# mpieva/mapping-iterative-assembler

Measured on AMD Instinct MI355X. Metric: reads aligned/sec per iteration (16.5kb mito ref, 100bp reads), higher is better.
Workload: dtype int32; 1 GPU; configs[1]: 1000000 synthetic 100 bp reads per GPU vs mt311 (16619 bp, circular), matrix flat; step = reiterate_assembly + pop_smp + cull + consensus; pass-1 coordinates = true positions; reads_per_gpu=1000000, total_reads=1000000, consensus_len=16619, bytes_per_read=182

## Files before the change

mapping-iterative-assembler_amd/csrc/mia_consensus_kernels.h:

```cpp
#pragma once
#include <hip/hip_runtime.h>
#include <stdint.h>

#include "ma_records.h"
#include "mia_kernels.h"
#include "mia_layout.h"

namespace mia {

struct TallyBuf {
  int32_t* tally;
  int32_t Lp;
  int32_t* gaps;
  uint64_t* events;
  int32_t* n_events;
  int32_t cap_events;
  uint32_t* flags;
};

struct RecGeom {
  int start_w, end, split, ncols_f, ncols_b;
};
MIA_HD inline RecGeom rec_geom(int as, int ae, int L) {
  RecGeom g;
// ... 684 lines not shown
        for (int m = 0; m < mult; m++) {
          int slot = BINNED ? atomicAdd(ev_cnt, 1) : TALLY_EV_CAP;
          if (slot < TALLY_EV_CAP) ev_buf[slot] = ev;
          else {
            const int e = atomicAdd(tb.n_events, 1);
            if (e < tb.cap_events) tb.events[e] = ev; else atomicOr(tb.flags, 1u);
          }
        }
      }
    }
  }
}

__global__ __launch_bounds__(256) void k_tally(ReadSet rs, RefInfo ref, const int32_t* pssm2, const uint8_t* drop_front,
                                                const uint8_t* drop_back, TallyBuf tb, const int32_t* rec_params, const int32_t* rec_actf) {
  const int lane = threadIdx.x & 63;
  const int64_t i = (int64_t)blockIdx.x * 4 + (threadIdx.x >> 6);
  if (i >= rs.n) return;
  tally_one_read<false>(__builtin_amdgcn_readfirstlane((int)i), lane, rs, ref, pssm2, drop_front, drop_back, tb, nullptr, 0, rec_params, rec_actf, nullptr, nullptr, nullptr);
}

constexpr int BUCKET_PER = 8;
__device__ __forceinline__ int bucket_of(const ReadSet& rs, int64_t i, int nb, int split) {
  return (min(rs.as[i] / TALLY_BUCKET, (nb >> split) - 1) << split) | (split ? (rs.rc[i] ? 1 : 0) : 0);
}
__device__ __forceinline__ bool bucket_takes(const ReadSet& rs, int64_t i) { return i < rs.n && rs.sk[i]; }
constexpr int SORT2_KEYS = 256;
__device__ __forceinline__ int sort2_key(const ReadSet& rs, int64_t i, int b, int split) {
  if (!(rs.status[i] & ST_DIAG) || rs.abr[i] != 0) return SORT2_KEYS - 1;
  const int k = rs.as[i] - (b >> split) * TALLY_BUCKET;
  return k < 0 ? 0 : (k >= SORT2_KEYS - 1 ? SORT2_KEYS - 2 : k);
}
__global__ __launch_bounds__(256) void k_bucket_count(ReadSet rs, int32_t nb, int32_t* count, int32_t* zero, int64_t zero_words, const int32_t* abort_if = nullptr,
                                                       int32_t split = 0) {
  if (abort_if && *abort_if != 0) return;
  extern __shared__ int32_t hist[];
  for (int b = threadIdx.x; b < nb; b += blockDim.x) hist[b] = 0;
  if (zero) for (int64_t k = (int64_t)blockIdx.x * 256 + threadIdx.x; k < zero_words; k += (int64_t)gridDim.x * 256) zero[k] = 0;
  __syncthreads();
  for (int k = 0; k < BUCKET_PER; k++) {
    const int64_t i = ((int64_t)blockIdx.x * BUCKET_PER + k) * 256 + threadIdx.x;
    if (bucket_takes(rs, i)) atomicAdd(&hist[bucket_of(rs, i, nb, split)], 1);
  }
  __syncthreads();
  for (int b = threadIdx.x; b < nb; b += blockDim.x) if (hist[b]) atomicAdd(&count[b], hist[b]);
}
__global__ __launch_bounds__(256) void k_bucket_scan(int32_t* count, int32_t nb, int32_t* off, int32_t* wgoff, int32_t* cursor, int32_t* wg_bucket, const int32_t* abort_if = nullptr,
                                                      int32_t chunk = TALLY_CHUNK) {
  if (abort_if && *abort_if != 0) return;
  __shared__ int32_t s_run[256], s_wg[256];
  const int t = threadIdx.x, per = (nb + 255) / 256, b0 = t * per, b1 = b0 + per < nb ? b0 + per : nb;
  int run = 0, wg = 0;
  for (int b = b0; b < b1; b++) { run += count[b]; wg += (count[b] + chunk - 1) / chunk; }
  s_run[t] = run; s_wg[t] = wg;
  __syncthreads();
  for (int o = 1; o < 256; o <<= 1) {
    const int a = t >= o ? s_run[t - o] : 0, c = t >= o ? s_wg[t - o] : 0;
    __syncthreads();
    s_run[t] += a; s_wg[t] += c;
    __syncthreads();
  }
  int r = s_run[t] - run, w = s_wg[t] - wg;
  for (int b = b0; b < b1; b++) {
    off[b] = r; wgoff[b] = w; cursor[b] = 0;
    const int cb = count[b];
    const int nw = (cb + chunk - 1) / chunk;
    for (int q = 0; q < nw; q++) reinterpret_cast<int4*>(wg_bucket)[w + q] = make_int4(b, r + q * chunk, min(r + (q + 1) * chunk, r + cb), 0);
    r += cb; w += nw;
    count[b] = 0;
  }
  if (t == 255) { off[nb] = s_run[255]; wgoff[nb] = s_wg[255]; }
// ... 936 lines not shown
      if (code < 4) atomicAdd(&t[(T_A + code) * Lp], 1);
      const int32_t* row = pm + d * 25 + code;
      atomicAdd(&t[T_SA * Lp], row[0]);
      atomicAdd(&t[T_SC * Lp], row[5]);
      atomicAdd(&t[T_SG * Lp], row[10]);
      atomicAdd(&t[T_ST * Lp], row[15]);
    }
    if (p > 0) atomicAdd(&t[T_SPAN * Lp], 1);
  }
}
__global__ void k_ma_ins_events(MaRecords mr, int64_t n_ins, const int32_t* ins_record, const int32_t* ins_pos, const int64_t* ins_off,
                                const char* ins_bases, TallyBuf tb) {
  const int64_t e = (int64_t)blockIdx.x * blockDim.x + threadIdx.x;
  if (e >= n_ins) return;
  const int r = ins_record[e], p = ins_pos[e];
  const int64_t o0 = mr.col_off[r];
  const int ncols = (int)(mr.col_off[r + 1] - o0);
  if (p <= 0 || p >= ncols) return;
  const int gc = mr.start[r] + p, d = (int)mr.smp[o0 + p] - 'A';
  if (gc >= tb.Lp || d < 0 || d > 2 * PSSM_DEPTH) { atomicOr(tb.flags, 2u); return; }
  const int len = (int)(ins_off[e + 1] - ins_off[e]);
  for (int j = 0; j < len && j < 1024; j++) {
    const int code = ma_code(ins_bases[ins_off[e] + j]);
    const int slot = atomicAdd(tb.n_events, 1);
    if (slot < tb.cap_events)
      tb.events[slot] = (uint64_t)(uint32_t)gc | ((uint64_t)j << 32) | ((uint64_t)(code == 5 ? 4 : code) << 42) | ((uint64_t)(d & 31) << 45) |
                        ((uint64_t)(mr.revcom[r] ? 1 : 0) << 50);
    else atomicOr(tb.flags, 1u);
  }
}

MIA_HD inline int64_t ins_words(int64_t cap) { return ((cap * 9 + 1) & ~(int64_t)1) + cap * 6; }
MIA_HD inline unsigned long long* ins_sc_of(int32_t* ins_tally, int64_t cap) { return reinterpret_cast<unsigned long long*>(ins_tally + ((cap * 9 + 1) & ~(int64_t)1)); }
__global__ void k_ins_tally(const uint64_t* events, int32_t n_events, const int32_t* pssm2, const int32_t* ins_off,
                            const int32_t* gaps, int32_t L, int32_t* ins_tally, int32_t cap, const int32_t* n_events_dev, int32_t cap_events, const int32_t* abort_if = nullptr) {
  if (abort_if && *abort_if != 0) return;
  if (n_events_dev) n_events = min(*n_events_dev, cap_events);
  for (int e = blockIdx.x * blockDim.x + threadIdx.x; e < n_events; e += gridDim.x * blockDim.x) {
  const uint64_t ev = events[e];
  const int gc = (int)(uint32_t)ev, j = (int)((ev >> 32) & 1023), code = (int)((ev >> 42) & 7), d = (int)((ev >> 45) & 31);
  const int rc = (int)((ev >> 50) & 1);
  if (gc <= 0 || gc >= L || j >= gaps[gc] || ins_off[gc] + j >= cap) continue;
  const int64_t sl = (int64_t)(ins_off[gc] + j);
  int32_t* t = ins_tally + sl * 9;
  unsigned long long* sc = ins_sc_of(ins_tally, cap) + sl * 3;
  const int32_t* row = pssm2 + (rc ? PSSM_WORDS : 0) + d * 25 + code;
  if (code < 4) atomicAdd(&t[code], 1);
  else atomicAdd(&sc[2], 1ull);
  atomicAdd(&sc[0], (unsigned long long)(((long long)row[5] << 32) + (long long)row[0]));
  atomicAdd(&sc[1], (unsigned long long)(((long long)row[15] << 32) + (long long)row[10]));
  }
}

__device__ __forceinline__ char call_base(int As, int Cs, int Gs, int Ts, int gapsn, int cov, int sA, int sC, int sG, int sT,
                                          int cons_code) {
  (void)As; (void)Cs; (void)Gs; (void)Ts;
  if (cov == 0) return 'N';
  if (((double)gapsn / (double)cov) >= (double)(50 / 100.0)) return '-';
  int top = sA, second = INT32_MIN;
  char base = 'A';
  if (sC >= top) { second = top; top = sC; base = 'C'; } else second = sC;
  if (sG >= top) { second = top; top = sG; base = 'G'; } else if (sG >= second) second = sG;
  if (sT >= top) { second = top; top = sT; base = 'T'; } else if (sT >= second) second = sT;
  if (cons_code == 2) return (top >= 0 || (top - 2400) > second) ? base : 'N';
  return (top >= -399) ? base : 'N';
}

__global__ void k_call_columns(const int32_t* tally, int32_t Lp, int32_t L, int cons_code, char* calls) {
  int p = blockIdx.x * blockDim.x + threadIdx.x;
  if (p >= L) return;
  calls[p] = call_base(tally[T_A * Lp + p], tally[T_C * Lp + p], tally[T_G * Lp + p], tally[T_T * Lp + p],
                       tally[T_GAP * Lp + p], tally[T_COV * Lp + p], tally[T_SA * Lp + p], tally[T_SC * Lp + p],
                       tally[T_SG * Lp + p], tally[T_ST * Lp + p], cons_code);
}
__device__ __forceinline__ void call_inserts_at(int p, const int32_t* tally, int32_t Lp, const int32_t* gaps, const int32_t* ins_off,
                                                int32_t* ins_tally, int cons_code, char* ins_calls, int32_t cap) {
  const int span = tally[T_SPAN * Lp + p];
  for (int j = 0; j < gaps[p] && ins_off[p] + j < cap; j++) {
    const int64_t sl = (int64_t)(ins_off[p] + j);
    int32_t* t = ins_tally + sl * 9;
    const unsigned long long* sc = ins_sc_of(ins_tally, cap) + sl * 3;
    const long long x0 = (long long)sc[0], x1 = (long long)sc[1];
    const int32_t sA = (int32_t)(uint32_t)x0, sC = (int32_t)((x0 - (long long)sA) >> 32), sG = (int32_t)(uint32_t)x1, sT = (int32_t)((x1 - (long long)sG) >> 32);
// ... 14 lines not shown
```

mapping-iterative-assembler_amd/csrc/mia_hip.hip:

```cpp
#include <hip/hip_runtime.h>
#include <atomic>
#include <hip/hip_ext.h>
#include <stdio.h>
#include <stdlib.h>
#include <string.h>

#include <algorithm>
#include <cmath>
#include <chrono>
#include <optional>
#include <string>
#include <thread>
#include <tuple>
#include <vector>

#include "../../include/mia_hip.h"
#include "dev_buf.h"
#include "dev_pool.h"
#include "mia_comm.h"
#include "mia_consensus_kernels.h"
#include "mia_kernels.h"
#include "bandx_kernels.h"
#include "align_route.h"
#include "pass1_route.h"
// ... 15 lines not shown
enum Stage { STG_TRACE = 0, STG_PLAIN, STG_FILTER, STG_BAND, STG_BX_PLAN, STG_BX_VALUES, STG_BX_TRACE, STG_TALLY, STG_PASS1, STG_MA_SELECT, STG_MA_RENDER, STG_MA_ACE_LAYOUT, STG_MA_ACE_RENDER, STG_MA_SAM_LAYOUT, STG_MA_SAM_RENDER, STG_MA_PROFILE, STG_MA_DEDUP_KEYS, STG_MA_DEDUP_SORT, STG_MA_DEDUP_RUNS, STG_MA_DEDUP_NEXT, STG_MA_DEDUP_ANCHORS, STG_MA_DEDUP_CLUSTERS, STG_MA_TALLY, STG_MA_COLS, STG_MA_ENDS, STG_COUNT };
static const char* const STAGE_NAMES[STG_COUNT] = {"k_align_quad", "k_align_quad_plain", "k_diag_filter", "k_band_align", "k_bx_plan",
                                                   "k_bx_values", "k_bx_trace", "k_tally_binned", "k_pass1", "k_ma_region_select",
                                                   "k_ma_region_render", "k_ma_ace_layout", "k_ma_ace_render", "k_ma_sam_layout",
                                                   "k_ma_sam_render", "k_ma_profile", "k_ma_dedup_keys", "k_ma_dedup_sort", "k_ma_dedup_runs",
                                                   "k_ma_dedup_next", "k_ma_dedup_anchors", "k_ma_dedup_clusters", "k_ma_tally", "k_ma_cols", "k_ma_ends"};

constexpr int OPEN_WGS = 1024;
constexpr int64_t OPEN_SLAB_BYTES = (int64_t)MAX_READ * 64 * 12;
constexpr int CTRL_BINS = 0;
constexpr int CTRL_HDR = (3 * N_BINS + 2 + 1) & ~1;
constexpr int CTRL_FILTER = CTRL_HDR + PH_WORDS;
constexpr int CTRL_LKN = CTRL_FILTER + 4, CTRL_CULLF = CTRL_LKN + 1, CTRL_NEV = CTRL_CULLF + 1, CTRL_TFLAGS = CTRL_NEV + 1;
constexpr int CTRL_GENN = CTRL_TFLAGS + 2;
constexpr int CTRL_BXC = (CTRL_GENN + 1 + 63) & ~63;
constexpr int CTRL_WORDS = CTRL_BXC + BXC_WORDS;
constexpr int CTRL_C0 = CTRL_BINS + 3 * N_BINS, CTRL_CN = CTRL_WORDS - CTRL_C0;

#ifdef MIA_HIP_ALT_PATHS
static inline const char* alt_env(const char* name) { return getenv(name); }
#define ALT_KERNEL(k) ((const void*)(k))
#else
static inline const char* alt_env(const char*) { return nullptr; }
#define ALT_KERNEL(k) ((const void*)nullptr)
#endif
static inline std::optional<int> alt_int(const char* name) {
  const char* v = alt_env(name);
  return v ? std::optional<int>(atoi(v)) : std::nullopt;
}

struct mia_hip_ctx {
  int device = 0;
  int cus = 1;
  std::string err;
  DevPool pool;
  unsigned char* h_pin = nullptr; static constexpr size_t PIN_BYTES = 1 << 20, PIN_MISC = 64 << 10;
  DevBuf<int32_t> d_ctrl;
  uint32_t dbg = 0;

  hipStream_t stream = nullptr;
  hipStream_t stream2 = nullptr; hipEvent_t ev_fork = nullptr, ev_join = nullptr;
  hipStream_t stream3 = nullptr; hipEvent_t ev_join3 = nullptr;
  uint32_t ext_events = 31u; bool align_end_signalled = false;
  bool spin_wait = true;
  uint32_t stage_mask = ~0u;
  struct StageTimer { std::vector<std::pair<hipEvent_t, hipEvent_t>> pending; double ms = 0; int64_t launches = 0; };
  StageTimer stg[STG_COUNT];
  std::vector<std::pair<hipEvent_t, hipEvent_t>> ev_free;

  DevBuf<int32_t> d_pssm;
  int max_abs = 0;
  int max_pos = 0;
  bool have_pssm = false;
  bool flat = false;
  PackSet packs;
  ReadSet rs{};
  DevBuf<uint8_t> d_packed; DevBuf<uint32_t> d_roff; DevBuf<uint16_t> d_len;
  DevBuf<uint8_t> d_rc, d_sk;
  DevBuf<int32_t> d_as, d_ae, d_score, d_refstart;
  DevBuf<int16_t> d_abr; DevBuf<uint32_t> d_status; DevBuf<int16_t> d_cols;
  int max_len = 0;
  int min_len = 0;
  std::vector<int32_t> h_len;
  DevBuf<uint64_t> d_rplanes; int rplane_words = 0;
  DevBuf<int32_t> d_umax; bool umax_valid = false;
  DevBuf<uint8_t> d_ref; int L = 0, wrap = 0; int explicit_win = 0; bool have_ref = false; bool aligned = false;
// ... 45 lines not shown
  DevBuf<int32_t> d_retry2;
  bool diag_scripts_missing = false;
  int64_t bx_seen = 0, bx_done[3] = {0, 0, 0};
  int64_t bx_launches = 0;
  uint32_t bx_last[BXC_COUNTERS] = {0};

  DevBuf<int64_t> d_slot, d_partial, d_total;
  DevBuf<uint8_t> d_slot_dropped, d_drop_f, d_drop_b; int64_t n_slots = 0;
  DevBuf<int64_t> d_back_slot;
  DevBuf<int64_t> d_front_slot0;
  DevBuf<int32_t> d_link_act;
  RecInfo ri{};
  DevBuf<int32_t> d_ri_flen, d_ri_blen, d_ri_actf, d_ri_trec;
  SlotInfo si{};
  DevBuf<int32_t> d_si_reclen, d_si_recact, d_si_mult; DevBuf<unsigned long long> d_si_writer;
  Links lk{};
  DevBuf<int64_t> d_lk_rec;
  int64_t* d_links_all = nullptr; int32_t n_links_all = 0;
  int32_t* d_n_links_all = nullptr; int64_t links_cap_all = 0; DevBuf<int32_t> d_n_links_gathered;
  DevBuf<int32_t> d_link_len;
  uint32_t* d_cull_flags = nullptr;
  DevBuf<uint32_t> d_cull_sync;
  DevBuf<unsigned long long> d_sums;
  int64_t read_base = 0;
  int64_t slot_base = 0;
  bool culled = false, links_applied = false;
  std::vector<DevBuf<int64_t>> owned_links;
  bool cull_scan = false, tail_scans = false;
  bool cull_with_records = true;
  int64_t pre_cull_records = 0, pre_cull_links = 0; bool pre_cull_valid = false;

  TallyBuf tb{}; DevBuf<int32_t> d_tb_tally, d_ins_off, d_ins_total; DevBuf<uint64_t> d_tb_events;
  DevBuf<int32_t> d_ins_tally; DevBuf<char> d_calls, d_ins_calls;
  int64_t ins_tally_cap = 0;
  int32_t n_events_host = 0; bool tallied = false;
  int64_t ins_total_host = 0;
  bool consensus_done = false;
  bool fake_event_overflow = false;
  bool no_linear_tally = false, sort2_unpacked = false;
  bool tally_linear = false;
  int tally_pk_bias = -1;
  int use_binned_tally = 1;
  DevBuf<int32_t> d_bucket, d_order;
  int bucket_clean_nb = -1;
  int buckets_queued = 0;
  bool no_side_buckets = false;
  DevBuf<int32_t> d_tally_slabs;
  DevBuf<int32_t> d_gen_list;
  bool tally_defer = true;
  bool tally_strand_split = true;
  bool tally_rall = true;
  bool tally_runs = true;
  DevBuf<int32_t> d_order2; DevBuf<uint8_t> d_okey; DevBuf<int32_t> d_sort2;

  bool in_iterate = false;
  const int32_t* abort_if = nullptr;
  bool spec_ok = false, spec_pending = false, spec_filtered = false, spec_bx = false, spec_plain = false;
  int64_t spec_redone = 0;
  bool no_spec = false;
  bool spec_force = false; DevBuf<int32_t> d_one;
  bool pend_encode = false; int32_t pend_L = 0, pend_wl = 0, pend_total = 0;
  bool zero_copy = true;
  const double* dev_cut = nullptr; DevBuf<double> d_cut_buf;
  DevBuf<char> d_ascii; const char* ascii_src = nullptr;
  DevBuf<char> d_cons;
  DevBuf<int32_t> d_cons_pos;
// ... 91 lines not shown
}
template <class T>
static int dev_alloc(mia_hip_ctx* ctx, DevBuf<T>& b, int64_t n) { return dev_nomem(ctx, b.alloc(n)); }
template <class T>
static int dev_ensure(mia_hip_ctx* ctx, DevBuf<T>& b, int64_t need, int64_t alloc_elems) { return dev_nomem(ctx, b.ensure(need, alloc_elems)); }
template <class T>
static int dev_ensure(mia_hip_ctx* ctx, DevBuf<T>& b, int64_t need) { return dev_nomem(ctx, b.ensure(need, need)); }

template <class T>
static int pool_take(mia_hip_ctx* ctx, PoolLease<T>& lease, size_t n) { return dev_nomem(ctx, lease.take(ctx->pool, n)); }

extern "C" const char* mia_hip_last_error(const mia_hip_ctx* ctx) { return ctx ? ctx->err.c_str() : "null context"; }

extern "C" int mia_hip_create(mia_hip_ctx** out, int device_index) {
  if (!out) return MIA_HIP_ERR_ARG;
  *out = nullptr;
  int ndev = 0;
  if (hipGetDeviceCount(&ndev) != hipSuccess || ndev <= 0) return MIA_HIP_ERR_DEVICE;
  if (device_index < 0 || device_index >= ndev) return MIA_HIP_ERR_ARG;
  mia_hip_ctx* ctx = new mia_hip_ctx();
  ctx->device = device_index;
  const unsigned evf = hipEventDisableTiming;
  if (hipSetDevice(device_index) != hipSuccess || hipStreamCreateWithFlags(&ctx->stream, hipStreamNonBlocking) != hipSuccess ||
      hipStreamCreateWithFlags(&ctx->stream2, hipStreamNonBlocking) != hipSuccess || hipStreamCreateWithFlags(&ctx->stream3, hipStreamNonBlocking) != hipSuccess ||
      hipEventCreateWithFlags(&ctx->ev_join3, evf) != hipSuccess ||
      hipEventCreateWithFlags(&ctx->ev_fork, evf) != hipSuccess || hipEventCreateWithFlags(&ctx->ev_join, evf) != hipSuccess) {
    delete ctx;
    return MIA_HIP_ERR_DEVICE;
  }
  {
    hipDeviceProp_t prop;
    if (hipGetDeviceProperties(&prop, device_index) != hipSuccess) { delete ctx; return MIA_HIP_ERR_DEVICE; }
    ctx->cus = prop.multiProcessorCount > 0 ? prop.multiProcessorCount : 1;
    ctx->grid_wgs = prop.multiProcessorCount * 32;
    ctx->quad_wgs = prop.multiProcessorCount * 16;
    read_alt_switches(ctx);
    if (const char* sw = getenv("MIA_HIP_SPIN_WAIT")) ctx->spin_wait = atoi(sw) != 0;
  }
  if (dev_alloc(ctx, ctx->d_pssm, 2 * PSSM_WORDS) || dev_alloc(ctx, ctx->d_ctrl, CTRL_WORDS) ||
      dev_alloc(ctx, ctx->d_total, 1) || dev_alloc(ctx, ctx->d_ins_total, 1) ||
      dev_alloc(ctx, ctx->d_bx_sub, 2 * BX_SUB_WORDS) || dev_alloc(ctx, ctx->d_bx_mrow, 2 * 31 * 4) || dev_alloc(ctx, ctx->d_bx_loss, BX_LOSS_WORDS) ||
      dev_alloc(ctx, ctx->d_bx_dl, BX_DL_WORDS) ||
      dev_alloc(ctx, ctx->d_cut_buf, 2)) {
    delete ctx;
    return MIA_HIP_ERR_NOMEM;
  }
  ctx->d_bins = ctx->d_ctrl + CTRL_BINS;
  ctx->d_plan_hdr = ctx->d_ctrl + CTRL_HDR;
  ctx->d_filter_n = reinterpret_cast<uint32_t*>(ctx->d_ctrl + CTRL_FILTER);
  ctx->lk.n = ctx->d_ctrl + CTRL_LKN;
  ctx->d_cull_flags = reinterpret_cast<uint32_t*>(ctx->d_ctrl + CTRL_CULLF);
  ctx->tb.n_events = ctx->d_ctrl + CTRL_NEV;
  ctx->tb.flags = reinterpret_cast<uint32_t*>(ctx->d_ctrl + CTRL_TFLAGS);
  ctx->d_bx_ctr = reinterpret_cast<uint32_t*>(ctx->d_ctrl + CTRL_BXC);
  if (hipMemset(ctx->d_ctrl, 0, CTRL_WORDS * 4) != hipSuccess) { delete ctx; return MIA_HIP_ERR_DEVICE; }
  {
    const int32_t one = 1;
    if (dev_alloc(ctx, ctx->d_one, 1) || hipMemcpy(ctx->d_one, &one, 4, hipMemcpyHostToDevice) != hipSuccess) { delete ctx; return MIA_HIP_ERR_DEVICE; }
    if (dev_alloc(ctx, ctx->d_prep_bar, 1) || hipMemset(ctx->d_prep_bar, 0, 4) != hipSuccess) { delete ctx; return MIA_HIP_ERR_DEVICE; }
  }
  if (hipHostMalloc((void**)&ctx->h_pin, mia_hip_ctx::PIN_BYTES, hipHostMallocDefault) != hipSuccess) ctx->h_pin = nullptr;
  if (ctx->h_pin) memset(ctx->h_pin, 0, mia_hip_ctx::PIN_MISC);
  else ctx->no_prep_fuse = true;
  *out = ctx;
  return MIA_HIP_OK;
}
// ... 1423 lines not shown
  return MIA_HIP_OK;
}

static int ensure_events(mia_hip_ctx* ctx, int64_t elems) {
  const int rc = dev_alloc(ctx, ctx->d_tb_events, elems);
  ctx->tb.events = ctx->d_tb_events;
  ctx->tb.cap_events = (int32_t)std::min<int64_t>(ctx->d_tb_events.cap, INT32_MAX);
  return rc;
}

static int ensure_tally(mia_hip_ctx* ctx) {
  const int Lp = ctx->L + 1;
  int rc = dev_ensure(ctx, ctx->d_tb_tally, (int64_t)(TALLY_WORDS + 1) * Lp + 256);
  rc |= dev_ensure(ctx, ctx->d_ins_off, Lp);
  rc |= dev_ensure(ctx, ctx->d_calls, Lp);
  if (rc) return MIA_HIP_ERR_NOMEM;
  if (!ctx->tb.events && ensure_events(ctx, std::min<int64_t>(ctx->rs.n * 32 + 4096, (int64_t)1 << 30))) return MIA_HIP_ERR_NOMEM;
  ctx->tb.tally = ctx->d_tb_tally;
  ctx->tb.Lp = Lp;
  ctx->tb.gaps = ctx->tb.tally + (size_t)TALLY_WORDS * Lp;
  return MIA_HIP_OK;
}

static bool tally_rall(const mia_hip_ctx* ctx) { return ctx->max_len > 128 && ctx->max_len <= 256 && ctx->tally_runs && ctx->tally_rall; }
static int tally_split(const mia_hip_ctx* ctx) {
  return (!ctx->tally_linear && ctx->tally_strand_split && (ctx->max_len <= 128 || tally_rall(ctx))) ? 1 : 0;
}
static int tally_nb(const mia_hip_ctx* ctx) { return (ctx->wrap / TALLY_BUCKET + 1) << tally_split(ctx); }
static bool tally_is_binned(const mia_hip_ctx* ctx) {
  const int nb = ctx->wrap / TALLY_BUCKET + 1;
  return ctx->rs.n > 0 && ctx->use_binned_tally && nb <= 4096 && ctx->max_abs <= 32767;
}
static int tally_chunk(const mia_hip_ctx* ctx) { return ctx->tally_linear ? TALLY_CHUNK_LINEAR : TALLY_CHUNK; }
static int bucket_launch(mia_hip_ctx* ctx, hipStream_t on) {
  int rc = ensure_tally(ctx);
  if (rc) return rc;
  const int Lp = ctx->tb.Lp;
  const int64_t tally_words = (int64_t)(TALLY_WORDS + 1) * Lp + 256;
  const int64_t n = ctx->rs.n;
  const int nb = tally_nb(ctx), split = tally_split(ctx);
  const int chunk = tally_chunk(ctx);
  const int grid = (int)(n / chunk) + nb + 1;
  if (4 * (nb + 1) + 4 * grid > ctx->d_bucket.cap) {
    if (dev_alloc(ctx, ctx->d_bucket, (int64_t)(4 * (nb + 1) + 4 * grid) * 2)) return MIA_HIP_ERR_NOMEM;
    ctx->bucket_clean_nb = -1;
  }
  if (!ctx->d_order && dev_alloc(ctx, ctx->d_order, n)) return MIA_HIP_ERR_NOMEM;
  int32_t *d_cnt = ctx->d_bucket, *d_off = d_cnt + (nb + 1), *d_wgoff = d_off + (nb + 1), *d_cur = d_wgoff + (nb + 1), *d_wgb = d_cur + (nb + 1);
  if (ctx->bucket_clean_nb != nb) { HIPCHK(hipMemsetAsync(d_cnt, 0, (size_t)(nb + 1) * 4, on)); ctx->bucket_clean_nb = nb; }
  const int gb = (int)((n + 256 * BUCKET_PER - 1) / (256 * BUCKET_PER));
  hipLaunchKernelGGL(k_bucket_count, dim3(gb), dim3(256), (size_t)nb * 4, on, ctx->rs, nb, d_cnt, ctx->tb.tally, tally_words, ctx->abort_if, split);
  hipLaunchKernelGGL(k_bucket_scan, dim3(1), dim3(256), 0, on, d_cnt, nb, d_off, d_wgoff, d_cur, d_wgb, ctx->abort_if, chunk);
  const bool sigb = on != ctx->stream && (ctx->ext_events & 16u);
  if (!split) launch_k(k_bucket_fill, dim3(gb), dim3(256), (size_t)nb * 8, on, sigb ? ctx->ev_join : nullptr, ctx->rs, nb, d_off, d_cur, ctx->d_order, ctx->abort_if, split, (uint8_t*)nullptr, 0);
  else {
    const int64_t words2 = (int64_t)nb * SORT2_KEYS * 2;
    if (dev_ensure(ctx, ctx->d_sort2, words2)) return MIA_HIP_ERR_NOMEM;
    if (!ctx->d_order2 && dev_alloc(ctx, ctx->d_order2, n)) return MIA_HIP_ERR_NOMEM;
    if (!ctx->d_okey && dev_alloc(ctx, ctx->d_okey, n + 64)) return MIA_HIP_ERR_NOMEM;
    HIPCHK(hipMemsetAsync(ctx->d_sort2, 0, (size_t)words2 * 4, on));
    const int32_t packed = (n < (1 << 24) && !ctx->sort2_unpacked) ? 1 : 0;
    hipLaunchKernelGGL(k_bucket_fill, dim3(gb), dim3(256), (size_t)nb * 8, on, ctx->rs, nb, (const int32_t*)d_off, d_cur, ctx->d_order, ctx->abort_if, split, ctx->d_okey, packed);
    hipLaunchKernelGGL(k_sort2_count, dim3(grid), dim3(256), 0, on, nb, (const int32_t*)d_wgoff, (const int32_t*)d_wgb, (const int32_t*)ctx->d_order, (const uint8_t*)ctx->d_okey, packed,
                       ctx->d_sort2, ctx->abort_if);
    launch_k(k_sort2_fill, dim3(grid), dim3(256), 0, on, sigb ? ctx->ev_join : nullptr, nb, (const int32_t*)d_off, (const int32_t*)d_wgoff, (const int32_t*)d_wgb,
             (const int32_t*)ctx->d_order, (const uint8_t*)ctx->d_okey, packed, (const int32_t*)ctx->d_sort2, ctx->d_sort2 + (int64_t)nb * SORT2_KEYS, ctx->d_order2, ctx->abort_if);
  }
  HIPCHK(hipGetLastError());
  if (on != ctx->stream && !sigb) HIPCHK(hipEventRecord(ctx->ev_join, on));
  ctx->buckets_queued = on != ctx->stream ? 2 : 1;
  return MIA_HIP_OK;
}

static int tally_launch(mia_hip_ctx* ctx) {
  if (!ctx->aligned) { ctx->err = "realign first"; return MIA_HIP_ERR_STATE; }
  if (!ctx->culled) { ctx->err = "cull first (the dropped bits and record parameters are its output)"; return MIA_HIP_ERR_STATE; }
  HIPCHK(hipSetDevice(ctx->device));
  int rc = ensure_tally(ctx);
  if (rc) return rc;
  const int Lp = ctx->tb.Lp;
  const int64_t tally_words = (int64_t)(TALLY_WORDS + 1) * Lp + 256;
  if (!ctx->in_iterate) HIPCHK(hipMemsetAsync(ctx->tb.n_events, 0, 8, ctx->stream));
  const int64_t n = ctx->rs.n;
  const bool binned = tally_is_binned(ctx);
// ... 209 lines not shown
```

mapping-iterative-assembler_amd/csrc/mia_hip_iterate.inc:

```

constexpr int PRE_WORDS = 8;
#define COLLCHK(call)                                                                                  \
  do {                                                                                                 \
    const int r_ = (call);                                                                             \
    if (r_ != MIA_HIP_OK) {                                                                            \
      const char* t_ = ctx->coll.error ? ctx->coll.error(ctx->coll.user) : nullptr;                    \
      ctx->err = std::string(#call) + ": " + (t_ && *t_ ? t_ : "collective failed");                   \
      return r_;                                                                                       \
    }                                                                                                  \
  } while (0)

static int comm_attach_table(mia_hip_ctx* ctx, const mia_hip_collectives& t) {
  if (dev_alloc(ctx, ctx->d_gather, (int64_t)PRE_WORDS * t.n_ranks)) return MIA_HIP_ERR_NOMEM;
  ctx->coll = t;
  ctx->coll_name = t.name ? t.name : "";
  ctx->coll.name = t.name ? ctx->coll_name.c_str() : nullptr;
  ctx->comm = true; ctx->comm_ranks = t.n_ranks; ctx->comm_rank = t.rank;
  ctx->h_gather.assign((size_t)PRE_WORDS * t.n_ranks, 0);
  ctx->ev_pad = 0;
  return MIA_HIP_OK;
}

extern "C" int mia_hip_comm_init(mia_hip_ctx* ctx, const void* id128, int32_t n_ranks, int32_t rank) {
  if (!ctx || !id128 || n_ranks < 1 || n_ranks > 256 || rank < 0 || rank >= n_ranks) return MIA_HIP_ERR_ARG;
// ... 145 lines not shown
      k += other(pq);
      if (pq >= DF_K) k -= other(pq - DF_K);
      if (pq >= DF_K - 1 && k <= BX_WILD) e += (int64_t)1 << (2 * k);
    }
    ctx->kh_entries = e > ((int64_t)1 << 24) ? 0 : e;
  }
  if (dev_ensure(ctx, ctx->d_ref, total, (int64_t)total * 2) || dev_ensure(ctx, ctx->d_ascii, L, (int64_t)L * 2)) return MIA_HIP_ERR_NOMEM;
  if (ctx->h_pin && (size_t)L <= mia_hip_ctx::PIN_BYTES - mia_hip_ctx::PIN_MISC) {
    HIPCHK(hipStreamSynchronize(ctx->stream));
    memcpy(ctx->h_pin + mia_hip_ctx::PIN_MISC, new_ref, (size_t)L);
    if (ctx->zero_copy) ctx->ascii_src = reinterpret_cast<const char*>(ctx->h_pin + mia_hip_ctx::PIN_MISC);
    else { HIPCHK(hipMemcpyAsync(ctx->d_ascii, ctx->h_pin + mia_hip_ctx::PIN_MISC, (size_t)L, hipMemcpyHostToDevice, ctx->stream)); ctx->ascii_src = ctx->d_ascii; }
  } else {
    HIPCHK(hipMemcpyAsync(ctx->d_ascii, new_ref, (size_t)L, hipMemcpyHostToDevice, ctx->stream));
    ctx->ascii_src = ctx->d_ascii;
  }
  ctx->pend_encode = true; ctx->pend_L = L; ctx->pend_wl = wl; ctx->pend_total = total;
  if (ctx->rs.n == 0) { encode_now(ctx); HIPCHK(hipGetLastError()); }
  const bool dbg_steps = alt_env("MIA_HIP_ITER_DEBUG") != nullptr;
  static const bool host_laps = getenv("MIA_HIP_TIMING") != nullptr;
  const auto lap_t0 = std::chrono::steady_clock::now();
  auto checkpoint = [&](const char* what) {
    if (dbg_steps) { hipError_t e = hipStreamSynchronize(ctx->stream); fprintf(stderr, "[mia_hip_iterate] %s: %s\n", what, hipGetErrorString(e)); fflush(stderr); }
    if (host_laps) fprintf(stderr, "[mia_hip_iterate host] %-20s %8.2f ms\n", what, std::chrono::duration<double, std::milli>(std::chrono::steady_clock::now() - lap_t0).count());
  };
  checkpoint("reference");
  ctx->L = L; ctx->wrap = wrap; ctx->have_ref = true; ctx->explicit_win = 0;
  const int64_t n = ctx->rs.n;
  const int W = ctx->comm_ranks;
  if (ctx->comm && n == 0) { ctx->err = "iterate: every rank of a sharded run needs reads"; return MIA_HIP_ERR_ARG; }
  if (ctx->comm && W > 256 - COMM_FLAG_SLOTS) { ctx->err = "iterate: more than 253 ranks"; return MIA_HIP_ERR_ARG; }
  ctx->in_iterate = true;
  ctx->deferred = true;
  ctx->spec_pending = false; ctx->abort_if = nullptr;
  ctx->spec_ok = !ctx->comm && n > 0 && !ctx->no_spec && (hard_cut > 0 || slope_intercept || ctx->min_len == ctx->max_len);
  const int rca = align_all(ctx);
  ctx->deferred = false;
  ctx->spec_ok = false;
  ctx->pend_encode = false;
  if (rca) { ctx->spec_pending = false; ctx->abort_if = nullptr; return rca; }
  checkpoint("realign");
  int64_t slot_base = 0, g_sums[5] = {0, 0, 0, 0, 0};
  std::vector<int64_t> link_counts((size_t)W, 0), n_of((size_t)W, n);
  if (ctx->comm) {
    g_sums[3] = INT32_MAX; g_sums[4] = INT32_MIN;
    for (int r = 0; r < W; r++) {
      const int64_t* q = ctx->h_gather.data() + (size_t)PRE_WORDS * r;
      g_sums[0] += q[0]; g_sums[1] += q[1]; g_sums[2] += q[2];
      g_sums[3] = std::min(g_sums[3], q[3]); g_sums[4] = std::max(g_sums[4], q[4]);
      if (r < ctx->comm_rank) slot_base += q[5];
      link_counts[(size_t)r] = q[6];
    }
  }
  double slope = 0, intercept = 0;
  const bool one_length = ctx->comm ? (g_sums[2] == 0 || g_sums[3] == g_sums[4]) : (ctx->min_len == ctx->max_len || n == 0);
  if (hard_cut > 0) {
  } else if (slope_intercept) {
    slope = slope_intercept[0]; intercept = slope_intercept[1];
  } else if (one_length) {
    const double zero = 0.0;
    slope = intercept = zero / zero;
  } else if (!ctx->comm) {
    std::vector<int32_t> score((size_t)n);
    HIPCHK(hipMemcpyAsync(score.data(), ctx->d_score, (size_t)n * 4, hipMemcpyDeviceToHost, ctx->stream));
    HIPCHK(hipStreamSynchronize(ctx->stream));
    mia_hip_score_cut(score.data(), ctx->h_len.data(), nullptr, n, &slope, &intercept);
// ... 94 lines not shown
    HIPCHK(hipGetLastError());
    return MIA_HIP_OK;
  };
  bool counted = false;
  if (ctx->comm) {
    if (ctx->fake_event_overflow)
      hipLaunchKernelGGL(k_or_u32, dim3(1), dim3(1), 0, ctx->stream, ctx->tb.flags, 1u);
    hipLaunchKernelGGL(k_put_rank_words, dim3(1), dim3(1), 0, ctx->stream, ctx->tb.gaps + Lp, (int32_t)ctx->comm_rank, (int32_t)W, (const int32_t*)ctx->tb.n_events,
                       ctx->tb.cap_events, (const uint32_t*)ctx->tb.flags, (const uint32_t*)ctx->d_cull_flags);
    COLLCHK(ctx->coll.all_reduce_i32(ctx->coll.user, ctx->tb.tally, (size_t)TALLY_WORDS * Lp, MIA_HIP_OP_SUM, ctx->stream));
    COLLCHK(ctx->coll.all_reduce_i32(ctx->coll.user, ctx->tb.gaps, (size_t)Lp + W + COMM_FLAG_SLOTS, MIA_HIP_OP_MAX, ctx->stream));
    counted = ctx->ev_pad <= 0;
    if (int rce = counted ? exchange_events_counted() : exchange_events_padded()) return rce;
  }
  const int64_t cons_cap = (int64_t)L + ctx->ins_tally_cap + 64;
  const int64_t res_bytes = (int64_t)CH_WORDS * 4 + cons_cap;
  if (dev_ensure(ctx, ctx->d_cons, res_bytes, res_bytes * 2) || dev_ensure(ctx, ctx->d_cons_pos, Lp, (int64_t)Lp * 2)) return MIA_HIP_ERR_NOMEM;
  const size_t need = (size_t)res_bytes;
  if (need > ctx->pin2_bytes) {
    if (ctx->h_pin2) (void)hipHostFree(ctx->h_pin2);
    ctx->h_pin2 = nullptr; ctx->pin2_bytes = 0;
    if (hipHostMalloc((void**)&ctx->h_pin2, need * 2, hipHostMallocDefault) != hipSuccess) { ctx->err = "hipHostMalloc"; return MIA_HIP_ERR_NOMEM; }
    ctx->pin2_bytes = need * 2;
  }
  int32_t* h_hdr = reinterpret_cast<int32_t*>(ctx->h_pin2);
  char* h_str = reinterpret_cast<char*>(ctx->h_pin2) + CH_WORDS * 4;
  auto consensus_tail = [&]() -> int {
    const int64_t cap = ctx->ins_tally_cap;
    int32_t* d_res = reinterpret_cast<int32_t*>(ctx->d_cons.p);
    const unsigned gl = (unsigned)((L + 255) / 256);
    const bool zc = ctx->zero_copy;
    const bool fused_scans = Lp <= (1 << 17) && !ctx->tail_scans;
    const unsigned glp = (unsigned)((Lp + 255) / 256);
    if (!fused_scans) {
      hipLaunchKernelGGL(k_excl_scan, dim3(1), dim3(1024), 0, ctx->stream, (const int32_t*)ctx->tb.gaps, Lp, 1, L, ctx->d_ins_off, ctx->d_ins_total, ctx->abort_if);
      hipLaunchKernelGGL(k_call_columns_z, dim3(gl), dim3(256), 0, ctx->stream, (const int32_t*)ctx->tb.tally, Lp, L, cons_code, ctx->d_calls, ctx->d_ins_tally, ins_words(cap), ctx->abort_if,
                         (const int32_t*)nullptr, (int32_t*)nullptr, (int32_t*)nullptr);
    } else
      hipLaunchKernelGGL(k_call_columns_z, dim3(glp > gl ? glp : gl), dim3(256), 0, ctx->stream, (const int32_t*)ctx->tb.tally, Lp, L, cons_code, ctx->d_calls, ctx->d_ins_tally, ins_words(cap), ctx->abort_if,
                         (const int32_t*)ctx->tb.gaps, ctx->d_ins_off, ctx->d_ins_total);
    if (cap > 0)
      hipLaunchKernelGGL(k_ins_tally, dim3(256), dim3(256), 0, ctx->stream, ctx->tb.events, 0, ctx->d_pssm, ctx->d_ins_off, ctx->tb.gaps, L, ctx->d_ins_tally,
                         (int32_t)cap, (const int32_t*)ctx->tb.n_events, ctx->tb.cap_events, ctx->abort_if);
    checkpoint("consensus kernels");
    hipLaunchKernelGGL(k_call_inserts_count, dim3(gl), dim3(256), 0, ctx->stream, (const int32_t*)ctx->tb.tally, Lp, L, (const int32_t*)ctx->tb.gaps,
                       (const int32_t*)ctx->d_ins_off, ctx->d_ins_tally, cons_code, (const char*)ctx->d_calls, ctx->d_ins_calls, (int32_t)cap,
                       (const int32_t*)ctx->d_ins_total, ctx->d_cons_pos, ctx->abort_if);
    if (!fused_scans) hipLaunchKernelGGL(k_excl_scan, dim3(1), dim3(1024), 0, ctx->stream, (const int32_t*)ctx->d_cons_pos, L, 0, L, ctx->d_cons_pos, d_res + CH_LEN, ctx->abort_if);
    hipLaunchKernelGGL(k_cons_scatter, dim3(gl), dim3(256), 0, ctx->stream, (const char*)ctx->d_calls, (const char*)ctx->d_ins_calls,
                       (const int32_t*)ctx->tb.gaps, (const int32_t*)ctx->d_ins_off, L, (int32_t)cap, (const int32_t*)ctx->d_ins_total,
                       (const int32_t*)ctx->d_cons_pos, d_res, (int32_t)cons_cap, (const int32_t*)ctx->tb.n_events, (const uint32_t*)ctx->tb.flags,
                       (const uint32_t*)ctx->d_cull_flags, ctx->abort_if, zc ? reinterpret_cast<int32_t*>(ctx->h_pin2) : (int32_t*)nullptr,
                       (const int32_t*)(ctx->d_ctrl + CTRL_C0), (int32_t)CTRL_CN, (zc && ctx->spec_pending) ? reinterpret_cast<int32_t*>(ctx->h_pin) : (int32_t*)nullptr,
                       fused_scans ? 1 : 0, ctx->comm ? (const int32_t*)(ctx->tb.gaps + Lp + W) : (const int32_t*)nullptr);
    HIPCHK(hipGetLastError());
    checkpoint("assemble");
    if (!zc) HIPCHK(hipMemcpyAsync(ctx->h_pin2, ctx->d_cons, need, hipMemcpyDeviceToHost, ctx->stream));
    if (ctx->comm && !counted) HIPCHK(hipMemcpyAsync(h_evc, ctx->tb.gaps + Lp, (size_t)W * 4, hipMemcpyDeviceToHost, ctx->stream));
    if (ctx->spin_wait) {
      hipError_t eq;
      while ((eq = hipStreamQuery(ctx->stream)) == hipErrorNotReady) {}
      HIPCHK(eq);
    } else HIPCHK(hipStreamSynchronize(ctx->stream));
    return MIA_HIP_OK;
  };
  if (int rct = consensus_tail()) return rct;
  if (ctx->h_pin) {
    uint32_t* stuck = reinterpret_cast<uint32_t*>(ctx->h_pin + (62 << 10));
    if (*stuck) {
      *stuck = 0;
      ctx->no_prep_fuse = true;
      ctx->err = "k_ref_prep: part of the launch never reached the grid barrier (device partitioned or compute units masked?); the iteration's results are void";
      return MIA_HIP_ERR_DEVICE;
    }
// ... 46 lines not shown
```

mapping-iterative-assembler_amd/csrc/mia_iter_kernels.h:

```cpp
#pragma once
#include <hip/hip_runtime.h>
#include <stdint.h>

namespace mia {

__device__ __forceinline__ uint8_t dev_base_code(char b) {
  return b == 'A' ? 0 : (b == 'C' ? 1 : (b == 'G' ? 2 : (b == 'T' ? 3 : 4)));
}

__global__ __launch_bounds__(256) void k_ref_encode(const char* ascii, int32_t L, int32_t wl, uint8_t* codes, int32_t total) {
  const int p = blockIdx.x * 256 + threadIdx.x;
  if (p >= total) return;
  codes[p] = p < L ? dev_base_code(ascii[p]) : (p < L + wl ? dev_base_code(ascii[p - L]) : (uint8_t)4);
}

struct RefPrep {
  const char* ascii; int32_t L, wl, total;
  uint8_t* codes;
  int32_t* ctrl; int32_t ctrl_words;
  uint32_t* kslot; int32_t* kovf; uint32_t kslots, kmask; int32_t kshift, kwild;
  int64_t plane_words; uint64_t *plo, *phi, *pok;
  int64_t nib_words; uint32_t* nib;
  uint32_t* bar; uint32_t bar_target;
  uint32_t* stuck;
// ... 131 lines not shown
  if (p < L && fits) {
    int32_t o = counts_in_pos ? my_pos : pos[p];
    if (p > 0 && ins_ok) for (int j = 0; j < gaps[p]; j++) { const char c = ins_calls[ins_off[p] + j]; if (cons_emits(c)) out[o++] = c; }
    const char c = calls[p];
    if (cons_emits(c)) out[o++] = c;
  }
  if (p == 0) {
    if (fits) out[len] = 0;
    dst[CH_LEN] = len;
    dst[CH_INS_TOTAL] = total; dst[CH_OVERFLOW] = (ins_ok && fits) ? 0 : 1;
    dst[CH_N_EVENTS] = n_events ? *n_events : 0;
    dst[CH_TALLY_FLAGS] = (tally_flags ? (int32_t)*tally_flags : 0) | ((peer_flags && peer_flags[0]) ? 1 : 0);
    dst[CH_CULL_FLAGS] = (cull_flags ? (int32_t)*cull_flags : 0) | ((peer_flags && peer_flags[1]) ? 4 : 0) | ((peer_flags && peer_flags[2]) ? 8 : 0);
  }
}

__global__ __launch_bounds__(256) void k_call_columns_z(const int32_t* tally, int32_t Lp, int32_t L, int cons_code, char* calls, int32_t* zero, int64_t zero_words, const int32_t* abort_if = nullptr,
                                                          const int32_t* gaps = nullptr, int32_t* ins_off = nullptr, int32_t* ins_total = nullptr) {
  if (abort_if && *abort_if != 0) return;
  const int p = blockIdx.x * 256 + threadIdx.x;
  if (gaps) {
    const bool last = (int)blockIdx.x == (Lp - 1) / 256;
    int32_t all = 0;
    const int32_t off = block_prefix_256(gaps, Lp, 1, L, last, &all);
    if (p < Lp) ins_off[p] = off;
    if (last && threadIdx.x == 0) *ins_total = all;
  }
  for (int64_t k = p; k < zero_words; k += (int64_t)gridDim.x * 256) zero[k] = 0;
  if (p >= L) return;
  calls[p] = call_base(tally[T_A * Lp + p], tally[T_C * Lp + p], tally[T_G * Lp + p], tally[T_T * Lp + p], tally[T_GAP * Lp + p], tally[T_COV * Lp + p],
                       tally[T_SA * Lp + p], tally[T_SC * Lp + p], tally[T_SG * Lp + p], tally[T_ST * Lp + p], cons_code);
}

__global__ __launch_bounds__(256) void k_call_inserts_count(const int32_t* tally, int32_t Lp, int32_t L, const int32_t* gaps, const int32_t* ins_off,
                                                              int32_t* ins_tally, int cons_code, const char* calls, char* ins_calls, int32_t ins_cap,
                                                              const int32_t* ins_total, int32_t* cnt, const int32_t* abort_if = nullptr) {
  if (abort_if && *abort_if != 0) return;
  const int p = blockIdx.x * 256 + threadIdx.x;
  if (p >= L) return;
  int32_t v = cons_emits(calls[p]) ? 1 : 0;
  if (p > 0) {
    call_inserts_at(p, tally, Lp, gaps, ins_off, ins_tally, cons_code, ins_calls, ins_cap);
    if (*ins_total <= ins_cap) for (int j = 0; j < gaps[p]; j++) v += cons_emits(ins_calls[ins_off[p] + j]) ? 1 : 0;
  }
  cnt[p] = v;
}

}
```

Measured before the change: 1.438 billion reads/s.

## Merge column calling and insertion tally into one kernel with per-block LDS prefix

Clearing the insertion tally moves into the earlier bucket-count kernel. The column-call pass and the insertion-tally pass are then fused into a single launch: extra blocks each rebuild the gap prefix sum in LDS (16-bit offsets) and apply insert events directly. This removes one kernel launch and the serial dependency on a global ins_off array. In exchange every insertion block redundantly scans the whole gaps array, and the fused path is gated on Lp and capacity bounds to keep the 16-bit offsets valid.

```diff
diff --git a/mapping-iterative-assembler_amd/csrc/mia_consensus_kernels.h b/mapping-iterative-assembler_amd/csrc/mia_consensus_kernels.h
--- a/mapping-iterative-assembler_amd/csrc/mia_consensus_kernels.h
+++ b/mapping-iterative-assembler_amd/csrc/mia_consensus_kernels.h
@@ -740,11 +740,12 @@
   return k < 0 ? 0 : (k >= SORT2_KEYS - 1 ? SORT2_KEYS - 2 : k);
 }
 __global__ __launch_bounds__(256) void k_bucket_count(ReadSet rs, int32_t nb, int32_t* count, int32_t* zero, int64_t zero_words, const int32_t* abort_if = nullptr,
-                                                       int32_t split = 0) {
+                                                       int32_t split = 0, int32_t* zero2 = nullptr, int64_t zero2_words = 0) {
   if (abort_if && *abort_if != 0) return;
   extern __shared__ int32_t hist[];
   for (int b = threadIdx.x; b < nb; b += blockDim.x) hist[b] = 0;
   if (zero) for (int64_t k = (int64_t)blockIdx.x * 256 + threadIdx.x; k < zero_words; k += (int64_t)gridDim.x * 256) zero[k] = 0;
+  if (zero2) for (int64_t k = (int64_t)blockIdx.x * 256 + threadIdx.x; k < zero2_words; k += (int64_t)gridDim.x * 256) zero2[k] = 0;
   __syncthreads();
   for (int k = 0; k < BUCKET_PER; k++) {
     const int64_t i = ((int64_t)blockIdx.x * BUCKET_PER + k) * 256 + threadIdx.x;
@@ -1747,23 +1748,33 @@
 
 MIA_HD inline int64_t ins_words(int64_t cap) { return ((cap * 9 + 1) & ~(int64_t)1) + cap * 6; }
 MIA_HD inline unsigned long long* ins_sc_of(int32_t* ins_tally, int64_t cap) { return reinterpret_cast<unsigned long long*>(ins_tally + ((cap * 9 + 1) & ~(int64_t)1)); }
+__device__ __forceinline__ void ins_tally_add(int32_t* ins_tally, int32_t cap, int64_t sl, int code, int32_t sa, int32_t sc_, int32_t sg, int32_t st) {
+  int32_t* t = ins_tally + sl * 9;
+  unsigned long long* sc = ins_sc_of(ins_tally, cap) + sl * 3;
+  if (code < 4) atomicAdd(&t[code], 1);
+  else atomicAdd(&sc[2], 1ull);
+  atomicAdd(&sc[0], (unsigned long long)(((long long)sc_ << 32) + (long long)sa));
+  atomicAdd(&sc[1], (unsigned long long)(((long long)st << 32) + (long long)sg));
+}
+__device__ __forceinline__ const int32_t* ins_event_row(uint64_t ev, const int32_t* pssm2) {
+  const int code = (int)((ev >> 42) & 7), d = (int)((ev >> 45) & 31), rc = (int)((ev >> 50) & 1);
+  return pssm2 + (rc ? PSSM_WORDS : 0) + d * 25 + code;
+}
+__device__ __forceinline__ void ins_tally_event(uint64_t ev, int32_t off, int gc, const int32_t* pssm2, const int32_t* gaps, int32_t* ins_tally, int32_t cap) {
+  const int j = (int)((ev >> 32) & 1023);
+  if (j >= gaps[gc] || off + j >= cap) return;
+  const int32_t* row = ins_event_row(ev, pssm2);
+  ins_tally_add(ins_tally, cap, (int64_t)(off + j), (int)((ev >> 42) & 7), row[0], row[5], row[10], row[15]);
+}
 __global__ void k_ins_tally(const uint64_t* events, int32_t n_events, const int32_t* pssm2, const int32_t* ins_off,
                             const int32_t* gaps, int32_t L, int32_t* ins_tally, int32_t cap, const int32_t* n_events_dev, int32_t cap_events, const int32_t* abort_if = nullptr) {
   if (abort_if && *abort_if != 0) return;
   if (n_events_dev) n_events = min(*n_events_dev, cap_events);
   for (int e = blockIdx.x * blockDim.x + threadIdx.x; e < n_events; e += gridDim.x * blockDim.x) {
-  const uint64_t ev = events[e];
-  const int gc = (int)(uint32_t)ev, j = (int)((ev >> 32) & 1023), code = (int)((ev >> 42) & 7), d = (int)((ev >> 45) & 31);
-  const int rc = (int)((ev >> 50) & 1);
-  if (gc <= 0 || gc >= L || j >= gaps[gc] || ins_off[gc] + j >= cap) continue;
-  const int64_t sl = (int64_t)(ins_off[gc] + j);
-  int32_t* t = ins_tally + sl * 9;
-  unsigned long long* sc = ins_sc_of(ins_tally, cap) + sl * 3;
-  const int32_t* row = pssm2 + (rc ? PSSM_WORDS : 0) + d * 25 + code;
-  if (code < 4) atomicAdd(&t[code], 1);
-  else atomicAdd(&sc[2], 1ull);
-  atomicAdd(&sc[0], (unsigned long long)(((long long)row[5] << 32) + (long long)row[0]));
-  atomicAdd(&sc[1], (unsigned long long)(((long long)row[15] << 32) + (long long)row[10]));
+    const uint64_t ev = events[e];
+    const int gc = (int)(uint32_t)ev;
+    if (gc <= 0 || gc >= L) continue;
+    ins_tally_event(ev, ins_off[gc], gc, pssm2, gaps, ins_tally, cap);
   }
 }
 
diff --git a/mapping-iterative-assembler_amd/csrc/mia_hip.hip b/mapping-iterative-assembler_amd/csrc/mia_hip.hip
--- a/mapping-iterative-assembler_amd/csrc/mia_hip.hip
+++ b/mapping-iterative-assembler_amd/csrc/mia_hip.hip
@@ -71,6 +71,7 @@
 struct mia_hip_ctx {
   int device = 0;
   int cus = 1;
+  int64_t lds_per_block = 65536;
   std::string err;
   DevPool pool;
   unsigned char* h_pin = nullptr; static constexpr size_t PIN_BYTES = 1 << 20, PIN_MISC = 64 << 10;
@@ -182,6 +183,7 @@
 
   TallyBuf tb{}; DevBuf<int32_t> d_tb_tally, d_ins_off, d_ins_total; DevBuf<uint64_t> d_tb_events;
   DevBuf<int32_t> d_ins_tally; DevBuf<char> d_calls, d_ins_calls;
+  bool ins_tally_clean = false;
   int64_t ins_tally_cap = 0;
   int32_t n_events_host = 0; bool tallied = false;
   int64_t ins_total_host = 0;
@@ -339,6 +341,7 @@
     hipDeviceProp_t prop;
     if (hipGetDeviceProperties(&prop, device_index) != hipSuccess) { delete ctx; return MIA_HIP_ERR_DEVICE; }
     ctx->cus = prop.multiProcessorCount > 0 ? prop.multiProcessorCount : 1;
+    ctx->lds_per_block = std::min<int64_t>((int64_t)prop.sharedMemPerBlock, 65536);
     ctx->grid_wgs = prop.multiProcessorCount * 32;
     ctx->quad_wgs = prop.multiProcessorCount * 16;
     read_alt_switches(ctx);
@@ -1828,9 +1831,16 @@
   return ctx->rs.n > 0 && ctx->use_binned_tally && nb <= 4096 && ctx->max_abs <= 32767;
 }
 static int tally_chunk(const mia_hip_ctx* ctx) { return ctx->tally_linear ? TALLY_CHUNK_LINEAR : TALLY_CHUNK; }
+constexpr int32_t TAIL_MERGE_MAX_LP = 32768;
+constexpr int64_t TAIL_MERGE_MAX_CAP = 65535;
+static bool tail_merge_ok(const mia_hip_ctx* ctx) {
+  return ctx->in_iterate && !ctx->tail_scans && ctx->tb.Lp <= TAIL_MERGE_MAX_LP && ctx->ins_tally_cap > 0 && ctx->ins_tally_cap <= TAIL_MERGE_MAX_CAP &&
+         (int64_t)ctx->tb.Lp * 2 + TAIL_LDS_STATIC <= ctx->lds_per_block;
+}
 static int bucket_launch(mia_hip_ctx* ctx, hipStream_t on) {
   int rc = ensure_tally(ctx);
   if (rc) return rc;
+  const bool clear_ins = tail_merge_ok(ctx);
   const int Lp = ctx->tb.Lp;
   const int64_t tally_words = (int64_t)(TALLY_WORDS + 1) * Lp + 256;
   const int64_t n = ctx->rs.n;
@@ -1845,7 +1855,9 @@
   int32_t *d_cnt = ctx->d_bucket, *d_off = d_cnt + (nb + 1), *d_wgoff = d_off + (nb + 1), *d_cur = d_wgoff + (nb + 1), *d_wgb = d_cur + (nb + 1);
   if (ctx->bucket_clean_nb != nb) { HIPCHK(hipMemsetAsync(d_cnt, 0, (size_t)(nb + 1) * 4, on)); ctx->bucket_clean_nb = nb; }
   const int gb = (int)((n + 256 * BUCKET_PER - 1) / (256 * BUCKET_PER));
-  hipLaunchKernelGGL(k_bucket_count, dim3(gb), dim3(256), (size_t)nb * 4, on, ctx->rs, nb, d_cnt, ctx->tb.tally, tally_words, ctx->abort_if, split);
+  hipLaunchKernelGGL(k_bucket_count, dim3(gb), dim3(256), (size_t)nb * 4, on, ctx->rs, nb, d_cnt, ctx->tb.tally, tally_words, ctx->abort_if, split,
+                     clear_ins ? ctx->d_ins_tally.p : (int32_t*)nullptr, clear_ins ? ins_words(ctx->ins_tally_cap) : (int64_t)0);
+  ctx->ins_tally_clean = clear_ins;
   hipLaunchKernelGGL(k_bucket_scan, dim3(1), dim3(256), 0, on, d_cnt, nb, d_off, d_wgoff, d_cur, d_wgb, ctx->abort_if, chunk);
   const bool sigb = on != ctx->stream && (ctx->ext_events & 16u);
   if (!split) launch_k(k_bucket_fill, dim3(gb), dim3(256), (size_t)nb * 8, on, sigb ? ctx->ev_join : nullptr, ctx->rs, nb, d_off, d_cur, ctx->d_order, ctx->abort_if, split, (uint8_t*)nullptr, 0);
diff --git a/mapping-iterative-assembler_amd/csrc/mia_hip_iterate.inc b/mapping-iterative-assembler_amd/csrc/mia_hip_iterate.inc
--- a/mapping-iterative-assembler_amd/csrc/mia_hip_iterate.inc
+++ b/mapping-iterative-assembler_amd/csrc/mia_hip_iterate.inc
@@ -201,6 +201,7 @@
   if (ctx->comm && W > 256 - COMM_FLAG_SLOTS) { ctx->err = "iterate: more than 253 ranks"; return MIA_HIP_ERR_ARG; }
   ctx->in_iterate = true;
   ctx->deferred = true;
+  ctx->ins_tally_clean = false;
   ctx->spec_pending = false; ctx->abort_if = nullptr;
   ctx->spec_ok = !ctx->comm && n > 0 && !ctx->no_spec && (hard_cut > 0 || slope_intercept || ctx->min_len == ctx->max_len);
   const int rca = align_all(ctx);
@@ -361,14 +362,21 @@
     const bool zc = ctx->zero_copy;
     const bool fused_scans = Lp <= (1 << 17) && !ctx->tail_scans;
     const unsigned glp = (unsigned)((Lp + 255) / 256);
-    if (!fused_scans) {
+    const bool merged = fused_scans && ctx->ins_tally_clean && tail_merge_ok(ctx);
+    ctx->ins_tally_clean = false;
+    if (merged) {
+      const unsigned n_call = glp > gl ? glp : gl;
+      hipLaunchKernelGGL(k_calls_ins_tally, dim3(n_call + TAIL_INS_BLOCKS), dim3(256), (size_t)Lp * 2, ctx->stream, (const int32_t*)ctx->tb.tally, Lp, L, cons_code, ctx->d_calls.p,
+                         (const int32_t*)ctx->tb.gaps, ctx->d_ins_off.p, ctx->d_ins_total.p, (int32_t)n_call, (const uint64_t*)ctx->tb.events, (const int32_t*)ctx->tb.n_events,
+                         ctx->tb.cap_events, (const int32_t*)ctx->d_pssm.p, ctx->d_ins_tally.p, (int32_t)cap, ctx->abort_if);
+    } else if (!fused_scans) {
       hipLaunchKernelGGL(k_excl_scan, dim3(1), dim3(1024), 0, ctx->stream, (const int32_t*)ctx->tb.gaps, Lp, 1, L, ctx->d_ins_off, ctx->d_ins_total, ctx->abort_if);
       hipLaunchKernelGGL(k_call_columns_z, dim3(gl), dim3(256), 0, ctx->stream, (const int32_t*)ctx->tb.tally, Lp, L, cons_code, ctx->d_calls, ctx->d_ins_tally, ins_words(cap), ctx->abort_if,
                          (const int32_t*)nullptr, (int32_t*)nullptr, (int32_t*)nullptr);
     } else
       hipLaunchKernelGGL(k_call_columns_z, dim3(glp > gl ? glp : gl), dim3(256), 0, ctx->stream, (const int32_t*)ctx->tb.tally, Lp, L, cons_code, ctx->d_calls, ctx->d_ins_tally, ins_words(cap), ctx->abort_if,
                          (const int32_t*)ctx->tb.gaps, ctx->d_ins_off, ctx->d_ins_total);
-    if (cap > 0)
+    if (cap > 0 && !merged)
       hipLaunchKernelGGL(k_ins_tally, dim3(256), dim3(256), 0, ctx->stream, ctx->tb.events, 0, ctx->d_pssm, ctx->d_ins_off, ctx->tb.gaps, L, ctx->d_ins_tally,
                          (int32_t)cap, (const int32_t*)ctx->tb.n_events, ctx->tb.cap_events, ctx->abort_if);
     checkpoint("consensus kernels");
diff --git a/mapping-iterative-assembler_amd/csrc/mia_iter_kernels.h b/mapping-iterative-assembler_amd/csrc/mia_iter_kernels.h
--- a/mapping-iterative-assembler_amd/csrc/mia_iter_kernels.h
+++ b/mapping-iterative-assembler_amd/csrc/mia_iter_kernels.h
@@ -187,6 +187,90 @@
                        tally[T_SA * Lp + p], tally[T_SC * Lp + p], tally[T_SG * Lp + p], tally[T_ST * Lp + p], cons_code);
 }
 
+constexpr int TAIL_INS_BLOCKS = 256;
+constexpr int TAIL_LDS_STATIC = 1280;
+__global__ __launch_bounds__(256) void k_calls_ins_tally(const int32_t* tally, int32_t Lp, int32_t L, int cons_code, char* calls, const int32_t* gaps, int32_t* ins_off,
+                                                           int32_t* ins_total, int32_t n_call, const uint64_t* events, const int32_t* n_events_dev, int32_t cap_events,
+                                                           const int32_t* pssm2, int32_t* ins_tally, int32_t cap, const int32_t* abort_if = nullptr) {
+  if (abort_if && *abort_if != 0) return;
+  const int t = threadIdx.x;
+  if ((int)blockIdx.x < n_call) {
+    const int p = blockIdx.x * 256 + t;
+    const bool last = (int)blockIdx.x == (Lp - 1) / 256;
+    int32_t all = 0;
+    const int32_t off = block_prefix_256(gaps, Lp, 1, L, last, &all);
+    if (p < Lp) ins_off[p] = off;
+    if (last && t == 0) *ins_total = all;
+    if (p >= L) return;
+    calls[p] = call_base(tally[T_A * Lp + p], tally[T_C * Lp + p], tally[T_G * Lp + p], tally[T_T * Lp + p], tally[T_GAP * Lp + p], tally[T_COV * Lp + p],
+                         tally[T_SA * Lp + p], tally[T_SC * Lp + p], tally[T_SG * Lp + p], tally[T_ST * Lp + p], cons_code);
+    return;
+  }
+  extern __shared__ __attribute__((aligned(16))) uint16_t s_off[];
+  __shared__ uint32_t s_base[256], s_wave[4];
+  auto sat16 = [](int32_t g) -> uint32_t { return g < 0 ? 0u : (g > 65535 ? 65535u : (uint32_t)g); };
+  auto gap_at = [&](int q, int32_t g) -> uint32_t { return (q >= 1 && q < L) ? sat16(g) : 0u; };
+  const int n_events = min(*n_events_dev, cap_events);
+  const int n_ins = (int)gridDim.x - n_call, e0 = ((int)blockIdx.x - n_call) * 256 + t;
+  const uint64_t ev0 = e0 < n_events ? events[e0] : 0ull;
+  const int gc0 = (int)(uint32_t)ev0;
+  const bool have0 = gc0 > 0 && gc0 < L;
+  int32_t g0 = 0, r0[4] = {0, 0, 0, 0};
+  if (have0) {
+    const int32_t* row = ins_event_row(ev0, pssm2);
+    g0 = gaps[gc0]; r0[0] = row[0]; r0[1] = row[5]; r0[2] = row[10]; r0[3] = row[15];
+  }
+  int q_done = 0;
+  if ((reinterpret_cast<uintptr_t>(gaps) & 15u) == 0u) {
+    const int n4 = Lp >> 2;
+#pragma unroll 8
+    for (int v = t; v < n4; v += 256) {
+      const int4 g = reinterpret_cast<const int4*>(gaps)[v];
+      const int q = v * 4;
+      *reinterpret_cast<uint2*>(s_off + q) = make_uint2(gap_at(q, g.x) | (gap_at(q + 1, g.y) << 16), gap_at(q + 2, g.z) | (gap_at(q + 3, g.w) << 16));
+    }
+    q_done = n4 * 4;
+  }
+#pragma unroll 8
+  for (int q = q_done + t; q < Lp; q += 256) s_off[q] = (uint16_t)gap_at(q, gaps[q]);
+  __syncthreads();
+  const int ch = ((Lp + 255) / 256) | 1, q0 = min(t * ch, (int)Lp), q1 = min(q0 + ch, (int)Lp);
+  uint32_t run = 0;
+  for (int q = q0; q < q1; q += 8) {
+    uint32_t v[8];
+#pragma unroll
+    for (int k = 0; k < 8; k++) v[k] = q + k < q1 ? (uint32_t)s_off[q + k] : 0u;
+#pragma unroll
+    for (int k = 0; k < 8; k++) {
+      if (q + k < q1) s_off[q + k] = (uint16_t)(run > 65535u ? 65535u : run);
+      run += v[k];
+    }
+  }
+  uint32_t inc = run;
+#pragma unroll
+  for (int o = 1; o < 64; o <<= 1) { const uint32_t u = __shfl_up(inc, o); if ((t & 63) >= o) inc += u; }
+  if ((t & 63) == 63) s_wave[t >> 6] = inc;
+  __syncthreads();
+  uint32_t base = inc - run;
+  for (int k = 0; k < (t >> 6); k++) base += s_wave[k];
+  s_base[t] = base;
+  __syncthreads();
+  auto off_of = [&](int gc) -> int32_t {
+    const uint32_t off = s_base[gc / ch] + (uint32_t)s_off[gc];
+    return (int32_t)(off > 65535u ? 65535u : off);
+  };
+  if (have0) {
+    const int j = (int)((ev0 >> 32) & 1023), off = off_of(gc0);
+    if (j < g0 && off + j < cap) ins_tally_add(ins_tally, cap, (int64_t)(off + j), (int)((ev0 >> 42) & 7), r0[0], r0[1], r0[2], r0[3]);
+  }
+  for (int e = e0 + n_ins * 256; e < n_events; e += n_ins * 256) {
+    const uint64_t ev = events[e];
+    const int gc = (int)(uint32_t)ev;
+    if (gc <= 0 || gc >= L) continue;
+    ins_tally_event(ev, off_of(gc), gc, pssm2, gaps, ins_tally, cap);
+  }
+}
+
 __global__ __launch_bounds__(256) void k_call_inserts_count(const int32_t* tally, int32_t Lp, int32_t L, const int32_t* gaps, const int32_t* ins_off,
                                                               int32_t* ins_tally, int cons_code, const char* calls, char* ins_calls, int32_t ins_cap,
                                                               const int32_t* ins_total, int32_t* cnt, const int32_t* abort_if = nullptr) {
```

Measured after the change: 1.442 billion reads/s, median of 2. About the same (+0.3%).
